# SysCV/LiDAR_snow_sim

Hardware: AMD Instinct MI355X
Metric: augmented points/s/GPU (64x2048 sweep, 2.5 mm/h); HBM roofline % -- value: rows resident in HBM when the clock starts (device-resident API: augment_batch on CUDA tensors); with H2D of the rows and D2H of the results inside the clock: value_pcie_inclusive (higher is better)
Workload: dtype f64

## Files before the change

lidar_snow_sim_amd/csrc/sg_common.h:

```cpp
#pragma once
#include <stddef.h>
#include <stdint.h>

#define SG_PI 3.141592653589793
#define SG_TWO_PI (2 * SG_PI)
#define SG_RBINS 1230
#define SG_NBINS 2048
#define SG_BIN_MARGIN 1e-6
#define SG_BEAM_MARGIN 1e-9
#define SG_TBL_STRIDE 16
#define SG_BLKREC 8
#define SG_HITS_UNDECIDED 0x40000000
#define SG_MAX_LASERS 256
#define SG_LCAP 63
#define SG_TILE 1024

struct SgEntry {
    double phi;
    double x, y, r;
    double t0, t1;
    double rho;
    uint32_t flags;
    uint32_t src;
};
// ... 51 lines not shown
    const void *srows;
    const int32_t *frame_unsorted;
    const SgTable *frame_tables;
    const SgLasers *las;
    const double *rgrid;
    double beam_div_deg;
    uint32_t *rec;
    uint32_t *rec_q;
    void *rng;
    int32_t *status;
    int32_t *tier_hint;
    unsigned long long *diff2;
    int32_t exact_math;
    int32_t n_cls;
    int32_t cls_cap[SG_MAX_CLASSES];
    const int32_t *seg_blk;
    const int64_t *seg_start;
    const int32_t *seg_cnt;
    const int32_t *seg_frame;
    const int32_t *seg_n;
    const int32_t *seg_of_blk;
    int64_t grid_blocks;
    int32_t q_chunk;
    int64_t blk_lo, blk_hi;
    const int32_t *chunk_blk;
    int32_t chunk;
    uint32_t *dq;
    int32_t *dq_g;
    uint16_t *dq_sc;
    unsigned long long *qn;
    int2_t *pw_items;
    int32_t *pw_count;
    int2_t *pw_items1;
    int32_t front_max;
    int64_t n_regions_ub;
    int32_t blk_rows;
    int32_t kp_lds_quarters;
    int64_t dq_n;
    int32_t *tier_list;
    int32_t *tier_info;
    int64_t tier_stride;
    int32_t *tier_sparse;
    int32_t *tn, *tbase;
    int32_t cls;
    int32_t work_lo, work_hi;
    int32_t work_hint;
    int32_t *redo_list;
    int32_t *redo_cnt;
    double *tq;
    uint16_t *tq_sc;
    int32_t tq_cap;
    double *ov;
    uint16_t *ov_sc;
    int32_t ov_cap;
    int32_t ov_list;
    double *h_lists;
    int32_t h_cap, h_lanes;
    int32_t *dbg_count;
    double *dbg_rj;
    double *dbg_ratio;
    int32_t dbg_cap;
};

struct SgFov {
    int32_t enabled;
    int32_t reserved_;
// ... 130 lines not shown
```

lidar_snow_sim_amd/csrc/sg_queue.h:

```cpp
#pragma once
#include "sg_beam.h"

#ifndef SG_DQ_ROW_HEADER
#define SG_DQ_ROW_HEADER 1
#endif
#if defined(__HIP_DEVICE_COMPILE__)
#define SG_DQ_RECORD(entries, w) (sg_gptr(entries) + ((w) & 0x3fffffffu))
#else
#define SG_DQ_RECORD(entries, w) ((entries) + ((w) & 0x3fffffffu))
#endif

__host__ __device__ __forceinline__ constexpr int sg_dq_hdr(int elem_size) { return SG_DQ_ROW_HEADER ? elem_size / 4 : 2; }
__host__ __device__ __forceinline__ constexpr int sg_dq_slot_words(int lmax, int hdr) { return 2 * hdr + lmax; }
__host__ __device__ __forceinline__ int64_t sg_dq_cell(int64_t slot, int plane, int lmax, int hdr)
{
    const int64_t group = (slot >> 6) * (int64_t)(64 * sg_dq_slot_words(lmax, hdr));
    const int c = (int)(slot & 63);
    return plane < 2 ? group + (int64_t)((plane * 64 + c) * hdr) : group + (int64_t)(128 * hdr + (plane - 2) * 64 + c);
}

template <typename T>
__host__ __device__ __forceinline__ void sg_dq_store_header(uint32_t *q, int64_t slot, int lmax, T d_t, T theta_t)
{
    constexpr int H = sg_dq_hdr((int)sizeof(T));
    using S = std::conditional_t<H == 2, double, float>;
    *reinterpret_cast<S *>(q + sg_dq_cell(slot, 0, lmax, H)) = (S)d_t;
    *reinterpret_cast<S *>(q + sg_dq_cell(slot, 1, lmax, H)) = (S)theta_t;
}
template <typename T>
__host__ __device__ __forceinline__ void sg_dq_store_word(uint32_t *q, int64_t slot, int lmax, int j, uint32_t w)
{
    q[sg_dq_cell(slot, 2 + j, lmax, sg_dq_hdr((int)sizeof(T)))] = w;
}

template <typename T>
__host__ __device__ __forceinline__ void sg_dq_load_header(const uint32_t *q, int64_t slot, int lmax, double &d, double &theta_c)
{
    constexpr int H = sg_dq_hdr((int)sizeof(T));
    using S = std::conditional_t<H == 2, double, float>;
    d = (double)*reinterpret_cast<const S *>(q + sg_dq_cell(slot, 0, lmax, H));
    theta_c = (double)*reinterpret_cast<const S *>(q + sg_dq_cell(slot, 1, lmax, H));
}
template <typename T>
__host__ __device__ __forceinline__ uint32_t sg_dq_load_word(const uint32_t *q, int64_t slot, int lmax, int j)
{
    return q[sg_dq_cell(slot, 2 + j, lmax, sg_dq_hdr((int)sizeof(T)))];
}

__host__ __device__ __forceinline__ void sg_dq_resolve(uint32_t w, const SgEntry *__restrict__ entries, double theta_r, double theta_l, double &a1, double &a2,
                                                       double &rho)
{
// ... 32 lines not shown
```

lidar_snow_sim_amd/csrc/snowgpu_batch.cpp:

```cpp
#include "sg_host.h"
#include "sg_launch.h"
#include "sg_queue.h"

static int sync_tables(snowgpu_ctx *ctx)
{
    if (!ctx->tables_dirty) return SNOWGPU_OK;
    const size_t n = std::max<size_t>(ctx->tables.size(), 1);
    if (n > ctx->d_tables_cap) {
        if (ctx->d_tables) { (void)hipStreamSynchronize(ctx->stream); (void)hipFree(ctx->d_tables); }
        HIPCHK(ctx, hipMalloc((void **)&ctx->d_tables, n * sizeof(SgTable)));
        ctx->d_tables_cap = n;
    }
    std::vector<SgTable> h(n);
    for (size_t i = 0; i < ctx->tables.size(); ++i) h[i] = ctx->tables[i].desc;
    HIPCHK(ctx, hipMemcpy(ctx->d_tables, h.data(), n * sizeof(SgTable), hipMemcpyHostToDevice));
    ctx->tables_dirty = false;
    return SNOWGPU_OK;
}

static void choose_tiers(const snowgpu_ctx *ctx, double beam_div_deg, int tiers[4], int *n_tiers)
{
    const double expect = (double)ctx->max_flakes * (beam_div_deg * (SG_PI / 180.0)) / SG_TWO_PI;
    int first = expect <= 24.0 ? 4 : (expect <= 48.0 ? 8 : (expect <= 96.0 ? 16 : SG_LCAP));
    if (ctx->first_tier_override == 4 || ctx->first_tier_override == 8 || ctx->first_tier_override == 16 ||
// ... 138 lines not shown
    const size_t regions = std::max<size_t>((size_t)b.n_frames * 256, n / q_chunk + 2);
    const size_t zero_words = 3 * regions + 2 * (size_t)b.n_frames + 8;
    ENSURE(ctx, ctx->qn, zero_words);
    ENSURE(ctx, ctx->tbase, SG_MAX_CLASSES * regions);
    bool seg_small = false;
    if (use_seg) {
        const int se = sg_launch_segments_small(b.frame_off, b.n_frames, ctx->tile_base.p, max_tiles, b.table_ids, R->h_las.n, (int)R->tables.size(), first_block,
                                                ctx->seg_blk.p, ctx->seg_start.p, ctx->seg_cnt.p, ctx->seg_frame.p, ctx->seg_n.p, ctx->seg_of_blk.p,
                                                ctx->chunk_blk.p, R->d_tables, ctx->frame_tables.p, ctx->qn.p, (int64_t)zero_words, st);
        if (se > 0) return fail(ctx, SNOWGPU_E_HIP, std::string("segment launch: ") + hipGetErrorString((hipError_t)se));
        seg_small = se == 0;
    }
    if (!seg_small) {
        HIPCHK(ctx, hipEventRecord(ctx->ev_fork, st));
        HIPCHK(ctx, hipStreamWaitEvent(s_aux, ctx->ev_fork, 0));
        int e = 0;
        if (!use_seg) e = sg_launch_resolve_tables(R->d_tables, (int)R->tables.size(), b.table_ids, n_ft, ctx->frame_tables.p, s_aux);
        if (e) return fail(ctx, SNOWGPU_E_HIP, std::string("table resolve launch: ") + hipGetErrorString((hipError_t)e));
        if (use_seg) {
            e = sg_launch_segments(b.frame_off, b.n_frames, ctx->tile_base.p, max_tiles, b.table_ids, R->h_las.n, (int)R->tables.size(), first_block,
                                   ctx->seg_tbl_cnt.p, ctx->seg_tbl_base.p, ctx->seg_blk.p, ctx->seg_start.p, ctx->seg_cnt.p, ctx->seg_frame.p,
                                   ctx->seg_n.p, ctx->seg_of_blk.p, ctx->chunk_blk.p, R->d_tables, ctx->frame_tables.p, s_aux);
            if (e) return fail(ctx, SNOWGPU_E_HIP, std::string("segment launch: ") + hipGetErrorString((hipError_t)e));
        }
        HIPCHK(ctx, hipEventRecord(ctx->ev_join, s_aux));
    }
    if (!b.perm) {
        int e = sg_launch_sort(b.rows, b.dtype, b.frame_off, b.n_frames, b.n_total, ctx->tile_hist.p, ctx->tile_base.p,
                               ctx->rank.p, ctx->keep.p, ctx->perm.p, b.status, max_tiles, nullptr, nullptr,
                               ctx->tile_unsorted.p, ctx->frame_unsorted.p, ctx->srows.p, b.want_perm ? 1 : 0, 2, st);
        if (e) return fail(ctx, SNOWGPU_E_HIP, std::string("sort launch: ") + hipGetErrorString((hipError_t)e));
    }
    ENSURE(ctx, ctx->rec, n);
    ENSURE(ctx, ctx->rec_q, n);
    ENSURE(ctx, ctx->rng, n * esz);
    ENSURE(ctx, ctx->keep, n);
    ENSURE(ctx, ctx->tier_list, n * (size_t)n_tiers);
    ENSURE(ctx, ctx->tier_sparse, n * (size_t)n_tiers);
    ENSURE(ctx, ctx->ctile_cnt, (size_t)b.n_frames * (size_t)max_tiles + 1);
    ENSURE(ctx, ctx->ctile_base, (size_t)b.n_frames * (size_t)max_tiles + 1);
    SgBeamArgs a{};
    a.rows = b.rows; a.frame_off = b.frame_off; a.n_frames = b.n_frames; a.n_total = b.n_total; a.perm = perm;
    a.srows = ctx->srows.p; a.frame_unsorted = ctx->frame_unsorted.p;
    a.uniform_rows = (b.uniform_rows > 0 && b.n_total < ((int64_t)1 << 31)) ? b.uniform_rows : 0;
    a.inv_uniform_rows = a.uniform_rows > 0 ? 1.0f / (float)a.uniform_rows : 0.0f;
    a.las = R->d_las; a.frame_tables = ctx->frame_tables.p;
    a.rgrid = R->d_rgrid; a.beam_div_deg = b.beam_div_deg; a.rec = ctx->rec.p; a.rec_q = ctx->rec_q.p;
    a.status = b.status;
    a.rng = ctx->rng.p;
    a.dbg_count = b.dbg_count; a.dbg_rj = b.dbg_rj; a.dbg_ratio = b.dbg_ratio; a.dbg_cap = b.dbg_cap;
    a.exact_math = R->exact_math;
    const int n_cls = n_tiers;
    const bool tier_rows = (R->tier_rows < 0 ? b.n_total <= ((int64_t)1 << 19) : R->tier_rows == 1) && R->tier_cap_override <= 0;
    const int h_lanes = 256;
    const int h_cap = (int)std::min<uint32_t>(std::max<uint32_t>(R->max_flakes, 64u), 8192u);
    a.n_cls = n_cls;
    for (int k = 0; k + 1 < n_cls; ++k) a.cls_cap[k] = tiers[k + 1];
    a.cls_cap[n_cls - 1] = h_cap;
    ENSURE(ctx, ctx->h_lists, (size_t)4 * (size_t)(h_cap + 1) * (size_t)h_lanes);
    a.h_lists = ctx->h_lists.p; a.h_cap = h_cap; a.h_lanes = h_lanes;
    a.tier_list = ctx->tier_list.p; a.tier_stride = b.n_total; a.tier_sparse = ctx->tier_sparse.p;
    if (tier_rows) {
        ENSURE(ctx, ctx->redo_list, n * (size_t)n_tiers);
        a.redo_list = ctx->redo_list.p;
    }
    const bool use_ov = tiers[0] < SG_OV_CAP && n_cls >= 2 && !tier_rows &&
                        R->tier_cap_override <= 0 && n * SG_OV_STRIDE * sizeof(double) <= ((size_t)40 << 30);
    int64_t tq_caps[SG_MAX_CLASSES] = {0, 0, 0, 0};
    for (int k = 0; k + 1 < n_cls && !tier_rows; ++k) {
        if (use_ov && tiers[k + 1] <= SG_OV_CAP) continue;
        tq_caps[k] = tier_queue_cap(R, tiers[k + 1], b.n_total);
        ENSURE(ctx, ctx->tq[k], ((size_t)tq_caps[k] + 64) * (3 * (size_t)tiers[k + 1] + 2));
        ENSURE(ctx, ctx->tq_sc[k], (size_t)tq_caps[k]);
    }
    a.q_chunk = (int32_t)q_chunk;
    {
        const size_t slot_words = (size_t)sg_dq_slot_words(tiers[0], sg_dq_hdr(b.dtype == 0 ? 4 : 8));
        if (n * slot_words * sizeof(uint32_t) > ((size_t)64 << 30))
            return fail(ctx, SNOWGPU_E_INVALID, "batch too large for the dict queue of this table density: split it");
        if (b.n_frames >= (1 << 22)) return fail(ctx, SNOWGPU_E_INVALID, "too many frames in one batch");
        ENSURE(ctx, ctx->dq, (n + 64) * slot_words);
        ENSURE(ctx, ctx->dq_g, n);
        ENSURE(ctx, ctx->dq_sc, n);
        if (!seg_small) HIPCHK(ctx, hipMemsetAsync(ctx->qn.p, 0, sizeof(unsigned long long) * zero_words, st));
        a.tn = (int32_t *)(ctx->qn.p + regions); a.tbase = ctx->tbase.p;
        a.diff2 = ctx->qn.p + 3 * regions;
        int32_t *small = (int32_t *)(ctx->qn.p + 3 * regions + (size_t)b.n_frames);
        a.tier_info = small; a.pw_count = small + 8; a.redo_cnt = small + 12;
        a.dq = ctx->dq.p; a.dq_g = ctx->dq_g.p; a.dq_sc = ctx->dq_sc.p; a.qn = ctx->qn.p; a.dq_n = b.n_total;
        const int lanes = first_block < 64 ? first_block : 64;
        a.n_regions_ub = use_seg ? (int64_t)b.n_frames * 256 : (b.n_total + a.q_chunk - 1) / a.q_chunk;
        a.blk_rows = first_block;
        a.kp_lds_quarters = 2;
        const size_t items_cap = n / (size_t)lanes + 2 * (size_t)a.n_regions_ub + 64;
        ENSURE(ctx, ctx->pw_items, 2 * items_cap);
        a.pw_items = ctx->pw_items.p;
        a.pw_items1 = (R->few > 0 && !b.dbg_count && lanes == 64) ? ctx->pw_items.p + items_cap : nullptr;
        a.front_max = a.pw_items1 ? std::min(R->few, std::min(3, tiers[0])) : 1;
    }
    if (use_ov) {
        ENSURE(ctx, ctx->ov, (n + 256) * SG_OV_STRIDE);
        ENSURE(ctx, ctx->ov_sc, n + 256);
        a.ov = ctx->ov.p; a.ov_sc = ctx->ov_sc.p; a.ov_cap = SG_OV_CAP;
    }
    if (use_seg) {
        a.seg_blk = ctx->seg_blk.p; a.seg_start = ctx->seg_start.p; a.seg_cnt = ctx->seg_cnt.p; a.seg_frame = ctx->seg_frame.p;
        a.seg_n = ctx->seg_n.p; a.seg_of_blk = ctx->seg_of_blk.p; a.chunk_blk = ctx->chunk_blk.p;
    }
    const bool few_first = a.pw_items1 && !serial && b.n_total > ((int64_t)1 << 19);
    bool heavy_tail = false;
    if (few_first && n_cls >= 3 && ctx->tier_hint_d) {
        const volatile int32_t *hint = ctx->tier_hint_h;
        long tail = 0;
        for (int k = 2; k < n_cls && k < SG_MAX_CLASSES; ++k) tail += hint[k];
        heavy_tail = R->heavy_tail < 0 ? (tail >= 4096 && tail * 22 > (long)hint[1]) : R->heavy_tail == 1;
        a.tier_hint = ctx->tier_hint_d;
    }
    if (!seg_small) HIPCHK(ctx, hipStreamWaitEvent(st, ctx->ev_join, 0));
    const bool timed = ctx->prof && ctx->ev_used < (int)ctx->ev_start.size();
    if (timed) { HIPCHK(ctx, hipEventRecord(ctx->ev_start[(size_t)ctx->ev_used], st)); ctx->prof_stream = st; }
    int e = 0;
    {
        const int64_t lin_blocks = (b.n_total + first_block - 1) / first_block;
        if (use_seg) {
            a.chunk = 0;
            a.grid_blocks = total_blocks_ub + b.max_frame / first_block + 2;
        } else {
            a.blk_lo = 0; a.blk_hi = lin_blocks;
            a.grid_blocks = lin_blocks;
        }
        e = sg_launch_beams(&a, b.dtype, tiers[0], 1, st);
// ... 144 lines not shown
```

lidar_snow_sim_amd/csrc/snowgpu_kernels.hip:

```cpp
#include <hip/hip_runtime.h>
#include <algorithm>
#include "sg_beam.h"
#include "sg_few.h"
#include "sg_queue.h"
#include "sg_kutil.h"
#include "sg_launch.h"

#ifndef SG_NB4
#define SG_NB4 4
#endif
#ifndef SG_KP_WIN
#define SG_KP_WIN 3
#endif
#ifndef SG_FP_WAVES
#define SG_FP_WAVES 6
#endif
#ifndef SG_FP_WAVES_SEG
#define SG_FP_WAVES_SEG 7
#endif
#ifndef SG_NB_TIERS
#define SG_NB_TIERS 4
#endif
#ifndef SG_KP_THREE_MAX
#define SG_KP_THREE_MAX 16
// ... 209 lines not shown
                tier_k = k;
                pending = true;
            }
        } else if (o.range_error) {
            atomicCAS(&a.status[0], 0, 4 );
            atomicCAS(&a.status[1], -1, (int32_t)g);
        }
    }
    if constexpr (!LIST) {
        if (__ballot(tier_k >= 0)) {
            for (int k = 0; k < a.n_cls; ++k) {
                const unsigned long long m = __ballot(tier_k == k);
                if (!m) continue;
                const int leader = __ffsll((long long)m) - 1;
                int base = 0;
                if ((tid & 63) == leader) base = atomicAdd(&a.tn[(int64_t)__builtin_amdgcn_readfirstlane(region) * SG_MAX_CLASSES + k], (int)__popcll(m));
                base = __shfl(base, leader);
                if (tier_k == k) a.tier_sparse[(int64_t)k * a.tier_stride + q_base + base + (int)__popcll(m & sg_lanemask_lt())] = (int32_t)g;
            }
        }
    }
    if constexpr (DICT) {
        auto hand_over = [&](uint32_t *q, int64_t slot) {
            sg_dq_store_header<T>(q, slot, LMAX, d_t, theta_t);
            const uint32_t *s_w = reinterpret_cast<const uint32_t *>(s_a1);
            if constexpr (LMAX <= 4) {
#pragma unroll
                for (int j = 0; j < LMAX; ++j)
                    if (j < L) sg_dq_store_word<T>(q, slot, LMAX, j, s_w[j * BLOCK + tid]);
            } else {
                for (int j = 0; j < L; ++j) sg_dq_store_word<T>(q, slot, LMAX, j, s_w[j * BLOCK + tid]);
            }
        };
        const bool front = o.has_power && L <= a.front_max, back = o.has_power && L > a.front_max;
        const unsigned long long mf = __ballot(front), mb = __ballot(back);
        if (mf | mb) {
            const int leader = __ffsll((long long)(mf | mb)) - 1;
            unsigned long long base = 0;
            if ((tid & 63) == leader)
                base = atomicAdd(&a.qn[__builtin_amdgcn_readfirstlane(region)], (unsigned long long)__popcll(mf) | ((unsigned long long)__popcll(mb) << 32));
            const unsigned blo = __shfl((unsigned)(base & 0xffffffffull), leader), bhi = __shfl((unsigned)(base >> 32), leader);
            if (o.has_power) {
                const int64_t slot = front ? q_base + (int)blo + (int)__popcll(mf & sg_lanemask_lt())
                                           : q_base + q_size - 1 - ((int)bhi + (int)__popcll(mb & sg_lanemask_lt()));
                hand_over(a.dq, slot);
                a.dq_g[slot] = (int32_t)g;
                a.dq_sc[slot] = (uint16_t)(L | (ch << 8));
                rec = SG_REC_SLOT | (uint32_t)slot;
            }
        }
    } else {
        constexpr int NB = LMAX <= 4 ? 4 : 8;
        if (o.has_power) {
            double best = 0.0;
            int k_best = 0;
            if (a.exact_math) sg_lane_power<BLOCK, true, NB, LMAX>(o.n_flakes, a.rgrid, s_a1, s_a2, s_rho, s_ratio, tid, best, k_best);
            else sg_lane_power<BLOCK, false, NB, LMAX>(o.n_flakes, a.rgrid, s_a1, s_a2, s_rho, s_ratio, tid, best, k_best);
            if constexpr (SgReal<T>::is_f32) d_t = sqrtf((px * px + py * py) + pz * pz);
            else d_t = sqrt((px * px + py * py) + pz * pz);
            sg_beam_decide((double)d_t, ch, a.las, best, k_best, o);
            rec = sg_pack_record(o);
        }
        sg_add_diff2(a.diff2, live, f, (long long)o.diff2);
    }
    if constexpr (DICT) {
        if (live && !pending && rec == 0u && act && a.rng) rec = rec_clear;
    }
    if (live && !pending) a.rec[g] = rec;
    } while (LIST && (chunk += stride) < work_n);
}

template <typename T, int LMAX>
__global__ __launch_bounds__(256, 4) void k_tier_scan_direct(SgBeamArgs a)
{
    constexpr int P = SG_QPLANES(LMAX);
    if constexpr (LMAX > 16) __builtin_amdgcn_s_setprio(3);
    const int n_las = a.las->n;
// ... 45 lines not shown
                a.dbg_rj[(int64_t)g * a.dbg_cap] = (double)d_t;
                a.dbg_ratio[(int64_t)g * a.dbg_cap] = sg_clear_beam_ratio(geo.theta_c, a.beam_div_deg);
            }
        } else {
            q[0] = (double)d_t; q[64] = geo.theta_c;
            a.tq_sc[slot] = (uint16_t)(hits | (ch << 8));
        }
    }
}

__device__ __forceinline__ bool sg_region(const SgBeamArgs &a, int r, int n_regions_ub, int64_t &q_base, int &q_size, int &f1)
{
    const int64_t lo = a.chunk_blk ? a.chunk_blk[a.chunk] : a.blk_lo, hi = a.chunk_blk ? a.chunk_blk[a.chunk + 1] : a.blk_hi;
    bool mine = false;
    q_base = 0; q_size = 0; f1 = 0;
    if (a.seg_blk) {
        if (r < a.seg_n[0]) {
            const int64_t b0 = a.seg_blk[r];
            mine = b0 >= lo && b0 < hi;
            if (mine) { q_base = a.seg_start[r]; q_size = a.seg_cnt[r]; f1 = (a.seg_frame[r] & 0x3fffff) + 1; }
        }
    } else if (r < n_regions_ub) {
        q_base = (int64_t)r * a.q_chunk;
        const int64_t b0 = q_base / a.blk_rows;
        mine = q_base < a.n_total && b0 >= lo && b0 < hi;
        if (mine) q_size = (int)(a.n_total - q_base < a.q_chunk ? a.n_total - q_base : a.q_chunk);
    }
    return mine;
}

__global__ __launch_bounds__(256) void k_power_plan(SgBeamArgs a, int lanes, int lanes_back, int n_regions_ub)
{
    const int r = blockIdx.x * 256 + threadIdx.x;
    int n_items = 0, nf = 0, nb = 0, q_size = 0, f1 = 0;
    int64_t q_base = 0;
    const bool mine = sg_region(a, r, n_regions_ub, q_base, q_size, f1);
    for (int k = 0; k < a.n_cls; ++k) {
        const int c = mine ? a.tn[(int64_t)r * SG_MAX_CLASSES + k] : 0;
        int inc = c;
        for (int o = 1; o < 64; o <<= 1) { const int v = __shfl_up(inc, o); if ((int)(threadIdx.x & 63) >= o) inc += v; }
        const int total = __shfl(inc, 63);
        int base = 0;
        if ((threadIdx.x & 63) == 63 && total > 0) base = atomicAdd(&a.tier_info[k], total);
        base = __shfl(base, 63) + inc - c;
        if (mine) a.tbase[(int64_t)r * SG_MAX_CLASSES + k] = base;
    }
    int n_one = 0;
    if (mine) {
        const unsigned long long c = a.qn[r];
        nf = (int)(c & 0xffffffffull); nb = (int)(c >> 32);
        n_one = (nf + lanes - 1) / lanes;
        n_items = (nb + lanes_back - 1) / lanes_back;
        if (!a.pw_items1) { n_items += n_one; n_one = 0; }
    }
    auto reserve = [&](int n, int32_t *counter) {
        int inc = n;
        for (int o = 1; o < 64; o <<= 1) { const int v = __shfl_up(inc, o); if ((int)(threadIdx.x & 63) >= o) inc += v; }
        const int total = __shfl(inc, 63);
        int b = 0;
        if ((threadIdx.x & 63) == 63 && total > 0) b = atomicAdd(counter, total);
        return __shfl(b, 63) + inc - n;
    };
    int base = reserve(n_items, a.pw_count);
    if (a.pw_items1) {
        int base1 = reserve(n_one, a.pw_count + 1);
        for (int k = 0; k < nf; k += lanes)
            a.pw_items1[base1++] = make_int2((int)(q_base + k), (nf - k < lanes ? nf - k : lanes) | (f1 << 10));
    } else {
        for (int k = 0; k < nf; k += lanes)
            a.pw_items[base++] = make_int2((int)(q_base + k), (nf - k < lanes ? nf - k : lanes) | (f1 << 10));
    }
    for (int k = 0; k < nb; k += lanes_back)
        a.pw_items[base++] = make_int2((int)(q_base + q_size - nb + k), (nb - k < lanes_back ? nb - k : lanes_back) | (f1 << 10));
}

__global__ __launch_bounds__(256) void k_tier_gather(SgBeamArgs a, int n_regions_ub)
{
    const int r = blockIdx.x * 4 + (int)(threadIdx.x >> 6), lane = (int)(threadIdx.x & 63);
    if (blockIdx.x == 0 && threadIdx.x < SG_MAX_CLASSES) a.status[2 + threadIdx.x] = a.tier_info[threadIdx.x];
    if (blockIdx.x == 0 && threadIdx.x < SG_MAX_CLASSES && a.tier_hint) a.tier_hint[threadIdx.x] = a.tier_info[threadIdx.x];
    if (blockIdx.x == 0 && threadIdx.x == 0 && a.tier_hint) a.tier_hint[SG_MAX_CLASSES] = (int32_t)((a.n_total >> 10) + 1);
    int q_size = 0, f1 = 0;
    int64_t q_base = 0;
    if (!sg_region(a, r, n_regions_ub, q_base, q_size, f1)) return;
    for (int k = 0; k < a.n_cls; ++k) {
        const int c = a.tn[(int64_t)r * SG_MAX_CLASSES + k];
        if (c == 0) continue;
        const int32_t *src = a.tier_sparse + (int64_t)k * a.tier_stride + q_base;
        int32_t *dst = a.tier_list + (int64_t)k * a.tier_stride + a.tbase[(int64_t)r * SG_MAX_CLASSES + k];
        for (int i = lane; i < c; i += 64) dst[i] = src[i];
    }
}

__device__ __forceinline__ const SgEntry *sg_dq_entries(const SgBeamArgs &a, int f, int ch)
{
    return a.frame_tables[(int64_t)f * a.las->n + ch].entries;
}

template <typename T, int LMAX, int BLOCK, bool LISTQ>
__device__ __forceinline__ void sg_kp_item(const SgBeamArgs &a, char *smem, const int ov_list, const int64_t work_off,
                                           const int start, const int cnt, const int item_f)
{
    constexpr int LANES = BLOCK < 64 ? BLOCK : 64;
    constexpr int WIN = BLOCK < 64 ? 1 : SG_KP_WIN;
    constexpr int P = SG_QPLANES(LMAX);
    double *s_a1 = (double *)smem;
// ... 223 lines not shown
    constexpr int THREADS = BLOCK < 64 ? 64 : BLOCK, WAVES = THREADS / 64, LANES = BLOCK < 64 ? BLOCK : 64;
    constexpr int WIN = BLOCK < 64 ? 1 : SG_KP_WIN;
    extern __shared__ __attribute__((aligned(16))) char smem[];
    if constexpr (LMAX > 16) __builtin_amdgcn_s_setprio(3);
    const int tid = threadIdx.x;
    int64_t work_n = 0, work_off = 0;
    int n_items;
    const int step = (int)gridDim.x * WAVES;
    int item_slots = LANES * WIN;
    if (LISTQ) {
        work_n = a.tier_info[a.cls];
        if (work_n > a.work_hi) work_n = a.work_hi;
        work_off = (int64_t)a.cls * a.tier_stride;
        if (WIN > 1 && work_n <= (int64_t)step * LANES) item_slots = LANES;
        n_items = (int)((work_n + item_slots - 1) / item_slots);
    } else {
        n_items = *a.pw_count;
    }
    for (int i = (int)blockIdx.x * WAVES + __builtin_amdgcn_readfirstlane(tid >> 6); i < n_items; i += step) {
        int start, cnt, item_f = -1;
        if (LISTQ) {
            start = i * item_slots;
            cnt = (int)(work_n - start < item_slots ? work_n - start : item_slots);
        } else {
            const int2 d = a.pw_items[i];
            start = __builtin_amdgcn_readfirstlane(d.x);
            const int dy = __builtin_amdgcn_readfirstlane(d.y);
            cnt = dy & 1023; item_f = (dy >> 10) - 1;
        }
        sg_kp_item<T, LMAX, BLOCK, LISTQ>(a, smem, a.ov_list, work_off, start, cnt, item_f);
    }
}

template <typename T, int N>
__global__ __launch_bounds__(256, 4) void k_power_few(SgBeamArgs a, int lmax)
{
    __shared__ double s_amp[N + 1][256], s_rho[N + 1][256], s_best[256];
    __shared__ int s_win[N + 1][256], s_zone[N + 1][256], s_k[256];
    __shared__ int s_mark[256];
    const int tid = (int)threadIdx.x, lane = tid & 63, wbase = tid & ~63;
    const int n_items = a.pw_count[1];
    const int step = (int)gridDim.x * 4;
    for (int i = (int)blockIdx.x * 4 + __builtin_amdgcn_readfirstlane(tid >> 6); i < n_items; i += step) {
        const int2 it = a.pw_items1[i];
        const int start = __builtin_amdgcn_readfirstlane(it.x), dy = __builtin_amdgcn_readfirstlane(it.y);
        const int cnt = dy & 1023, item_f = (dy >> 10) - 1;
        const bool live = lane < cnt;
        const int64_t slot = (int64_t)start + lane;
        SgBeamOut o;
        o.overflow = 0; o.range_error = 0; o.diff2 = 0.0; o.has_power = 0; o.n_flakes = 0; o.n_hits = 0; o.label = 0; o.new_i = 0; o.k_best = 0;
        int f = 0, ch = 0, S = 0, g = 0;
        SgFew<N> P{};
        int zone[N + 1], n = 0;
#pragma unroll
        for (int z = 0; z <= N; ++z) zone[z] = 0;
        if (live) {
            const unsigned sc = a.dq_sc[slot];
            double d, tc;
            sg_dq_load_header<T>(a.dq, slot, lmax, d, tc);
            uint32_t w[N];
#pragma unroll
            for (int j = 0; j < N; ++j) w[j] = sg_dq_load_word<T>(a.dq, slot, lmax, j);
            ch = (int)(sc >> 8);
            g = a.dq_g[slot];
            f = item_f >= 0 ? item_f : sg_frame_of(a, g);
            const SgEntry *ent = sg_dq_entries(a, f, ch);
            double th_r, th_l, a1[N], a2[N], rho[N];
            sg_beam_limits(tc, a.beam_div_deg, th_r, th_l);
            sg_dq_resolve_all<N>(w, (int)(sc & 255u), ent, th_r, th_l, a1, a2, rho);
            S = sg_few_prep<T, N>(d, tc, (int)(sc & 255u), a1, a2, rho, ch, a.las, a.beam_div_deg, P, o);
            if (S) {
                int ka, kb;
                sg_few_zone<N, 0>(P, 0.0, ka, kb);
                if (kb >= ka) { zone[0] = ka | ((kb - ka + 1) << 16); n += kb - ka + 1; }
                if constexpr (N >= 2) { sg_few_zone<N, 1>(P, 0.0, ka, kb); if (kb >= ka) { zone[1] = ka | ((kb - ka + 1) << 16); n += kb - ka + 1; } }
                if constexpr (N >= 3) { sg_few_zone<N, 2>(P, 0.0, ka, kb); if (kb >= ka) { zone[2] = ka | ((kb - ka + 1) << 16); n += kb - ka + 1; } }
                sg_few_zone<N, N>(P, 0.0, ka, kb);
// ... 48 lines not shown
                sm = a.exact_math ? sg_few_bin<true, N>(amp, rho, k0, k1, s_amp[N][col], s_rho[N][col], tw & 0xffff, (int)((unsigned)tw >> 16), k, a.rgrid)
                                  : sg_few_bin<false, N>(amp, rho, k0, k1, s_amp[N][col], s_rho[N][col], tw & 0xffff, (int)((unsigned)tw >> 16), k, a.rgrid);
                kk = k; oo = ow;
            }
            sg_fold_runs(sm, kk, oo);
            const int on = sg_dpp<0x130, 0xf>(oo, oo);
            if (valid && (lane == 63 || on != oo)) {
                volatile double *vb = s_best;
                volatile int *vk = s_k;
                const int col = wbase + oo;
                const double b0 = vb[col];
                const int kc = vk[col];
                if (sm > b0 || (sm == b0 && kk < kc)) { vb[col] = sm; vk[col] = kk; }
            }
        }
        asm volatile("s_waitcnt lgkmcnt(0)" ::: "memory");
        if (live) {
            uint32_t rec = 0;
            if (S) {
                const double best = ((volatile double *)s_best)[tid];
                const int k_best = ((volatile int *)s_k)[tid];
                if (o.range_error) {
                    atomicCAS(&a.status[0], 0, 4 );
                    atomicCAS(&a.status[1], -1, g);
                }
                sg_beam_decide(P.d, ch, a.las, best, k_best, o);
                rec = sg_pack_record(o);
            }
            a.rec_q[slot] = rec;
        }
        sg_add_diff2(a.diff2, live, f, live ? (long long)o.diff2 : 0);
        asm volatile("s_waitcnt lgkmcnt(0)" ::: "memory");
    }
}

template <typename T>
__global__ __launch_bounds__(64) void k_beams_huge(SgBeamArgs a)
{
    const int tid = (int)(blockIdx.x * 64 + threadIdx.x);
    const int rstride = a.h_lanes;
    const size_t col = (size_t)(a.h_cap + 1) * (size_t)a.h_lanes;
    double *s_a1 = a.h_lists, *s_a2 = s_a1 + col, *s_rho = s_a2 + col, *s_ratio = s_rho + col;
    const int n_las = a.las->n;
    int64_t work_n = a.tier_info[a.cls];
    const int64_t work_off = (int64_t)a.cls * a.tier_stride;
    int64_t chunk = (int64_t)blockIdx.x * 64;
    if (chunk >= work_n) return;
    do {
    const bool live = chunk + threadIdx.x < work_n;
    int64_t g = 0;
    int f = 0;
    SgBeamOut o;
    o.overflow = 0; o.range_error = 0; o.diff2 = 0.0; o.has_power = 0; o.n_flakes = 0; o.n_hits = 0; o.label = 0; o.new_i = 0; o.k_best = 0;
    if (live) {
        g = a.tier_list[work_off + chunk + threadIdx.x];
        f = sg_frame_of(a, g);
        const T *row = sg_row<T>(a, f, g);
        const T px = row[0], py = row[1], pz = row[2];
        const int ch = (int)row[4];
        const SgTable tab = a.frame_tables[(int64_t)f * n_las + ch];
        int32_t *dc = a.dbg_count ? a.dbg_count + g : nullptr;
        double *drj = a.dbg_count ? a.dbg_rj + g * a.dbg_cap : nullptr;
        double *dra = a.dbg_count ? a.dbg_ratio + g * a.dbg_cap : nullptr;
        sg_beam<T, 0, 0>(px, py, pz, ch, tab, a.las, a.beam_div_deg, s_a1, s_a2, s_rho, s_ratio, tid, o, a.dbg_cap, dc, drj,
                                dra, a.exact_math != 0, rstride, a.h_cap);
        uint32_t rec = 0;
// ... 44 lines not shown
    if (blocks == 0) return 0;
    hipLaunchKernelGGL((k_beams<T, LMAX, BLOCK, LIST, DICT, SEG>), dim3(blocks), dim3(THREADS), lds, st, *a);
    SG_CHECK_LAUNCH();
    return 0;
}

template <typename T, int LMAX, int BLOCK, bool LISTQ>
static int launch_power_t(const SgBeamArgs *a, hipStream_t st, bool plan_only = false, hipEvent_t ev_few = nullptr, int which = 3)
{
    const size_t lds = sizeof(double) * ((size_t)BLOCK * ((SG_KP_THREE_MAX > 0 && LMAX <= SG_KP_THREE_MAX && LMAX >= SG_KP_THREE_MIN) ? 3 : 4) * (LMAX + 1));
    static bool attr_set[64] = {};
    if (int e = sg_set_lds(k_power<T, LMAX, BLOCK, LISTQ>, lds, attr_set)) return e;
    constexpr int THREADS = BLOCK < 64 ? 64 : BLOCK, LANES = BLOCK < 64 ? BLOCK : 64;
    const int cus = sg_cu_count();
    unsigned per_cu = (unsigned)std::min<size_t>(32 * 64 / THREADS, std::max<size_t>(1, (size_t)(160 * 1024) / lds));
    if (!LISTQ && a->kp_lds_quarters > 0 && a->kp_lds_quarters < 4) per_cu = std::max(1u, per_cu * (unsigned)a->kp_lds_quarters / 4u);
    int64_t blocks = (int64_t)cus * per_cu;
    int64_t items_ub = LISTQ ? ((int64_t)a->work_hi + LANES - 1) / LANES : (a->n_total + LANES - 1) / LANES + 2 * a->n_regions_ub;
    if (LISTQ && a->work_hint > 0) items_ub = std::min<int64_t>(items_ub, (4 * (int64_t)a->work_hint + LANES - 1) / LANES + 8);
    blocks = std::min<int64_t>(blocks, (items_ub + THREADS / 64 - 1) / (THREADS / 64));
    if (blocks <= 0) return 0;
    if (!LISTQ) {
        const unsigned pg = (unsigned)((a->n_regions_ub + 255) / 256);
        if (pg == 0) return 0;
        const int64_t back_est = a->n_total / 10;
        const int lanes_back = (BLOCK < 64 || back_est <= (int64_t)blocks * (THREADS / 64) * LANES * 5 / 2) ? LANES : LANES * SG_KP_WIN;
        if (plan_only) {
            hipLaunchKernelGGL(k_power_plan, dim3(pg), dim3(256), 0, st, *a, LANES, lanes_back, (int)a->n_regions_ub);
            SG_CHECK_LAUNCH();
            return 0;
        }
        if (a->pw_items1 && (which & 1)) {
            hipStream_t s1 = st;
            const unsigned g1 = (unsigned)std::min<int64_t>((int64_t)cus * 4, (a->n_total / LANES + a->n_regions_ub + 3) / 4);
            if (g1 > 0) {
                if (a->front_max == 1) hipLaunchKernelGGL((k_power_few<T, 1>), dim3(g1), dim3(256), 0, s1, *a, LMAX);
                else if (a->front_max == 2) hipLaunchKernelGGL((k_power_few<T, 2>), dim3(g1), dim3(256), 0, s1, *a, LMAX);
                else hipLaunchKernelGGL((k_power_few<T, 3>), dim3(g1), dim3(256), 0, s1, *a, LMAX);
            }
            SG_CHECK_LAUNCH();
            if (ev_few && hipEventRecord(ev_few, st) != hipSuccess) return (int)hipGetLastError();
        }
    }
    if (!(which & 2)) return 0;
    hipLaunchKernelGGL((k_power<T, LMAX, BLOCK, LISTQ>), dim3((unsigned)blocks), dim3(THREADS), lds, st, *a);
    SG_CHECK_LAUNCH();
    return 0;
}

extern "C" int sg_launch_tier_scan(const SgBeamArgs *a, int dtype, int lmax, void *stream)
{
    const int64_t n = (int64_t)a->work_hi - a->work_lo;
    if (n <= 0) return 0;
    int64_t want = (n + 255) / 256;
    if (a->work_hint > 0) want = std::min<int64_t>(want, (4 * (int64_t)a->work_hint + 255) / 256 + 8);
    const unsigned blocks = (unsigned)std::min<int64_t>(want, (int64_t)sg_cu_count() * 8);
    return sg_by_dtype_tier<false>(dtype, lmax, [&](auto t, auto tier) {
        hipLaunchKernelGGL((k_tier_scan_direct<decltype(t), decltype(tier)::LMAX>), dim3(blocks), dim3(256), 0, (hipStream_t)stream, *a);
        SG_CHECK_LAUNCH();
        return 0;
    });
}

extern "C" int sg_beams_block(int lmax)
{
    return sg_by_tier<true>(lmax, [](auto tier) { return decltype(tier)::BLOCK; });
}

extern "C" int sg_launch_beams(const SgBeamArgs *a, int dtype, int lmax, int direct, void *stream)
{
    hipStream_t st = (hipStream_t)stream;
// ... 44 lines not shown
```

Baseline: 10.39 billion.

## Split dict queue into one-flake and few-flake lists for specialized power kernels

Beams whose front list holds one scatterer are now queued separately from those with two or three, using a second queue region (dq_n2 offset) and a three-way packed counter. The plan kernel emits separate work-item lists, and k_power_few processes single-flake items with the N=1 code path instead of the wider N=2/3 path. This avoids spending wider per-beam work and LDS on beams that need only one scatterer. The cost is roughly double the queue and rec_q allocations, extra packing logic, and either an extra launch or a combined kernel.

Result: no change. 10.45 billion (median of 6 runs) (+0.6%).

```diff
diff --git a/lidar_snow_sim_amd/csrc/sg_common.h b/lidar_snow_sim_amd/csrc/sg_common.h
--- a/lidar_snow_sim_amd/csrc/sg_common.h
+++ b/lidar_snow_sim_amd/csrc/sg_common.h
@@ -107,6 +107,8 @@
     int2_t *pw_items;
     int32_t *pw_count;
     int2_t *pw_items1;
+    int2_t *pw_items_one;
+    int64_t dq_n2;
     int32_t front_max;
     int64_t n_regions_ub;
     int32_t blk_rows;
diff --git a/lidar_snow_sim_amd/csrc/sg_queue.h b/lidar_snow_sim_amd/csrc/sg_queue.h
--- a/lidar_snow_sim_amd/csrc/sg_queue.h
+++ b/lidar_snow_sim_amd/csrc/sg_queue.h
@@ -17,6 +17,55 @@
     const int64_t group = (slot >> 6) * (int64_t)(64 * sg_dq_slot_words(lmax, hdr));
     const int c = (int)(slot & 63);
     return plane < 2 ? group + (int64_t)((plane * 64 + c) * hdr) : group + (int64_t)(128 * hdr + (plane - 2) * 64 + c);
+}
+
+#ifndef SG_FEW_SPLIT
+#define SG_FEW_SPLIT 1
+#endif
+enum { SG_DQ_ONE = 0, SG_DQ_FEW = 1, SG_DQ_BACK = 2 };
+#define SG_DQ_SPLIT_BITS 21
+struct SgDqCounts { int one, few, back; };
+
+__host__ __device__ __forceinline__ constexpr int64_t sg_dq_n2(int64_t n_total) { return (n_total + 63) & ~(int64_t)63; }
+__host__ __device__ __forceinline__ constexpr int64_t sg_dq_split_base(bool items1, int front_max, int64_t n_total)
+{
+    return (SG_FEW_SPLIT && items1 && front_max >= 2 && sg_dq_n2(n_total) + n_total + 64 < ((int64_t)1 << 31)) ? sg_dq_n2(n_total) : 0;
+}
+__host__ __device__ __forceinline__ constexpr int64_t sg_dq_slots(int64_t dq_n2, int64_t n_total) { return dq_n2 > 0 ? dq_n2 + n_total : n_total; }
+__host__ __device__ __forceinline__ constexpr bool sg_dq_split(int64_t dq_n2, int q_size) { return dq_n2 > 0 && q_size < (1 << SG_DQ_SPLIT_BITS); }
+__host__ __device__ __forceinline__ constexpr int sg_dq_kind(bool split, int L, int front_max)
+{
+    return L > front_max ? SG_DQ_BACK : (split && L >= 2 ? SG_DQ_FEW : SG_DQ_ONE);
+}
+__host__ __device__ __forceinline__ constexpr unsigned long long sg_dq_pack(bool split, int n_one, int n_few, int n_back)
+{
+    return split ? (unsigned long long)n_one | ((unsigned long long)n_few << SG_DQ_SPLIT_BITS) | ((unsigned long long)n_back << (2 * SG_DQ_SPLIT_BITS))
+                 : (unsigned long long)(n_one + n_few) | ((unsigned long long)n_back << 32);
+}
+__host__ __device__ __forceinline__ SgDqCounts sg_dq_unpack(bool split, unsigned long long w)
+{
+    constexpr unsigned long long M = (1ull << SG_DQ_SPLIT_BITS) - 1ull;
+    SgDqCounts c;
+    if (split) { c.one = (int)(w & M); c.few = (int)((w >> SG_DQ_SPLIT_BITS) & M); c.back = (int)((w >> (2 * SG_DQ_SPLIT_BITS)) & M); }
+    else { c.one = (int)(w & 0xffffffffull); c.few = 0; c.back = (int)(w >> 32); }
+    return c;
+}
+__host__ __device__ __forceinline__ int64_t sg_dq_place(int kind, int64_t q_base, int q_size, int64_t dq_n2, int index)
+{
+    return kind == SG_DQ_BACK ? q_base + q_size - 1 - index : (kind == SG_DQ_FEW ? dq_n2 + q_base + index : q_base + index);
+}
+struct SgDqItem { int64_t start; int count; };
+__host__ __device__ __forceinline__ int sg_dq_items(int kind, const SgDqCounts &c, int lanes, int lanes_back)
+{
+    return kind == SG_DQ_BACK ? (c.back + lanes_back - 1) / lanes_back : ((kind == SG_DQ_FEW ? c.few : c.one) + lanes - 1) / lanes;
+}
+__host__ __device__ __forceinline__ SgDqItem sg_dq_item(int kind, const SgDqCounts &c, int64_t q_base, int q_size, int64_t dq_n2, int lanes, int lanes_back, int i)
+{
+    const int per = kind == SG_DQ_BACK ? lanes_back : lanes, n = kind == SG_DQ_BACK ? c.back : (kind == SG_DQ_FEW ? c.few : c.one), k = i * per;
+    SgDqItem it;
+    it.start = kind == SG_DQ_BACK ? q_base + q_size - n + k : (kind == SG_DQ_FEW ? dq_n2 + q_base + k : q_base + k);
+    it.count = n - k < per ? n - k : per;
+    return it;
 }
 
 template <typename T>
diff --git a/lidar_snow_sim_amd/csrc/snowgpu_batch.cpp b/lidar_snow_sim_amd/csrc/snowgpu_batch.cpp
--- a/lidar_snow_sim_amd/csrc/snowgpu_batch.cpp
+++ b/lidar_snow_sim_amd/csrc/snowgpu_batch.cpp
@@ -194,7 +194,6 @@
         if (e) return fail(ctx, SNOWGPU_E_HIP, std::string("sort launch: ") + hipGetErrorString((hipError_t)e));
     }
     ENSURE(ctx, ctx->rec, n);
-    ENSURE(ctx, ctx->rec_q, n);
     ENSURE(ctx, ctx->rng, n * esz);
     ENSURE(ctx, ctx->keep, n);
     ENSURE(ctx, ctx->tier_list, n * (size_t)n_tiers);
@@ -207,7 +206,7 @@
     a.uniform_rows = (b.uniform_rows > 0 && b.n_total < ((int64_t)1 << 31)) ? b.uniform_rows : 0;
     a.inv_uniform_rows = a.uniform_rows > 0 ? 1.0f / (float)a.uniform_rows : 0.0f;
     a.las = R->d_las; a.frame_tables = ctx->frame_tables.p;
-    a.rgrid = R->d_rgrid; a.beam_div_deg = b.beam_div_deg; a.rec = ctx->rec.p; a.rec_q = ctx->rec_q.p;
+    a.rgrid = R->d_rgrid; a.beam_div_deg = b.beam_div_deg; a.rec = ctx->rec.p;
     a.status = b.status;
     a.rng = ctx->rng.p;
     a.dbg_count = b.dbg_count; a.dbg_rj = b.dbg_rj; a.dbg_ratio = b.dbg_ratio; a.dbg_cap = b.dbg_cap;
@@ -238,27 +237,33 @@
     a.q_chunk = (int32_t)q_chunk;
     {
         const size_t slot_words = (size_t)sg_dq_slot_words(tiers[0], sg_dq_hdr(b.dtype == 0 ? 4 : 8));
-        if (n * slot_words * sizeof(uint32_t) > ((size_t)64 << 30))
+        const int lanes = first_block < 64 ? first_block : 64;
+        const bool few_kernel = R->few > 0 && !b.dbg_count && lanes == 64;
+        a.front_max = few_kernel ? std::min(R->few, std::min(3, tiers[0])) : 1;
+        a.dq_n2 = sg_dq_split_base(few_kernel, a.front_max, b.n_total);
+        const size_t q_slots = (size_t)sg_dq_slots(a.dq_n2, b.n_total);
+        if (q_slots * slot_words * sizeof(uint32_t) > ((size_t)64 << 30))
             return fail(ctx, SNOWGPU_E_INVALID, "batch too large for the dict queue of this table density: split it");
         if (b.n_frames >= (1 << 22)) return fail(ctx, SNOWGPU_E_INVALID, "too many frames in one batch");
-        ENSURE(ctx, ctx->dq, (n + 64) * slot_words);
-        ENSURE(ctx, ctx->dq_g, n);
-        ENSURE(ctx, ctx->dq_sc, n);
+        ENSURE(ctx, ctx->dq, (q_slots + 64) * slot_words);
+        ENSURE(ctx, ctx->dq_g, q_slots);
+        ENSURE(ctx, ctx->dq_sc, q_slots);
+        ENSURE(ctx, ctx->rec_q, q_slots);
+        a.rec_q = ctx->rec_q.p;
         if (!seg_small) HIPCHK(ctx, hipMemsetAsync(ctx->qn.p, 0, sizeof(unsigned long long) * zero_words, st));
         a.tn = (int32_t *)(ctx->qn.p + regions); a.tbase = ctx->tbase.p;
         a.diff2 = ctx->qn.p + 3 * regions;
         int32_t *small = (int32_t *)(ctx->qn.p + 3 * regions + (size_t)b.n_frames);
         a.tier_info = small; a.pw_count = small + 8; a.redo_cnt = small + 12;
         a.dq = ctx->dq.p; a.dq_g = ctx->dq_g.p; a.dq_sc = ctx->dq_sc.p; a.qn = ctx->qn.p; a.dq_n = b.n_total;
-        const int lanes = first_block < 64 ? first_block : 64;
-        a.n_regions_ub = use_seg ? (int64_t)b.n_frames * 256 : (b.n_total + a.q_chunk - 1) / a.q_chunk;
+        a.n_regions_ub =use_seg ? (int64_t)b.n_frames * 256 : (b.n_total + a.q_chunk - 1) / a.q_chunk;
         a.blk_rows = first_block;
         a.kp_lds_quarters = 2;
         const size_t items_cap = n / (size_t)lanes + 2 * (size_t)a.n_regions_ub + 64;
-        ENSURE(ctx, ctx->pw_items, 2 * items_cap);
+        ENSURE(ctx, ctx->pw_items, (a.dq_n2 > 0 ? 3 : 2) * items_cap);
         a.pw_items = ctx->pw_items.p;
-        a.pw_items1 = (R->few > 0 && !b.dbg_count && lanes == 64) ? ctx->pw_items.p + items_cap : nullptr;
-        a.front_max = a.pw_items1 ? std::min(R->few, std::min(3, tiers[0])) : 1;
+        a.pw_items1 = few_kernel ? ctx->pw_items.p + items_cap : nullptr;
+        a.pw_items_one = a.dq_n2 > 0 ? ctx->pw_items.p + 2 * items_cap : nullptr;
     }
     if (use_ov) {
         ENSURE(ctx, ctx->ov, (n + 256) * SG_OV_STRIDE);
diff --git a/lidar_snow_sim_amd/csrc/snowgpu_kernels.hip b/lidar_snow_sim_amd/csrc/snowgpu_kernels.hip
--- a/lidar_snow_sim_amd/csrc/snowgpu_kernels.hip
+++ b/lidar_snow_sim_amd/csrc/snowgpu_kernels.hip
@@ -265,17 +265,21 @@
                 for (int j = 0; j < L; ++j) sg_dq_store_word<T>(q, slot, LMAX, j, s_w[j * BLOCK + tid]);
             }
         };
-        const bool front = o.has_power && L <= a.front_max, back = o.has_power && L > a.front_max;
-        const unsigned long long mf = __ballot(front), mb = __ballot(back);
-        if (mf | mb) {
-            const int leader = __ffsll((long long)(mf | mb)) - 1;
+        const bool split = sg_dq_split(a.dq_n2, q_size);
+        const int kind = o.has_power ? sg_dq_kind(split, L, a.front_max) : -1;
+        const unsigned long long mk = __ballot(kind >= 0);
+        if (mk) {
+            const unsigned long long mf = __ballot(kind == SG_DQ_FEW), mb = __ballot(kind == SG_DQ_BACK), mo = mk & ~(mf | mb);
+            const int leader = __builtin_amdgcn_readfirstlane(__ffsll((long long)mk) - 1);
             unsigned long long base = 0;
             if ((tid & 63) == leader)
-                base = atomicAdd(&a.qn[__builtin_amdgcn_readfirstlane(region)], (unsigned long long)__popcll(mf) | ((unsigned long long)__popcll(mb) << 32));
-            const unsigned blo = __shfl((unsigned)(base & 0xffffffffull), leader), bhi = __shfl((unsigned)(base >> 32), leader);
+                base = atomicAdd(&a.qn[__builtin_amdgcn_readfirstlane(region)], sg_dq_pack(split, (int)__popcll(mo), (int)__popcll(mf), (int)__popcll(mb)));
+            const SgDqCounts before = sg_dq_unpack(split, ((unsigned long long)(unsigned)__builtin_amdgcn_readlane((int)(base >> 32), leader) << 32)
+                                                              | (unsigned)__builtin_amdgcn_readlane((int)(base & 0xffffffffull), leader));
             if (o.has_power) {
-                const int64_t slot = front ? q_base + (int)blo + (int)__popcll(mf & sg_lanemask_lt())
-                                           : q_base + q_size - 1 - ((int)bhi + (int)__popcll(mb & sg_lanemask_lt()));
+                const unsigned long long mine = kind == SG_DQ_BACK ? mb : (kind == SG_DQ_FEW ? mf : mo);
+                const int index = (kind == SG_DQ_BACK ? before.back : (kind == SG_DQ_FEW ? before.few : before.one)) + (int)__popcll(mine & sg_lanemask_lt());
+                const int64_t slot = sg_dq_place(kind, q_base, q_size, a.dq_n2, index);
                 hand_over(a.dq, slot);
                 a.dq_g[slot] = (int32_t)g;
                 a.dq_sc[slot] = (uint16_t)(L | (ch << 8));
@@ -387,7 +391,7 @@
 __global__ __launch_bounds__(256) void k_power_plan(SgBeamArgs a, int lanes, int lanes_back, int n_regions_ub)
 {
     const int r = blockIdx.x * 256 + threadIdx.x;
-    int n_items = 0, nf = 0, nb = 0, q_size = 0, f1 = 0;
+    int n_items = 0, q_size = 0, f1 = 0;
     int64_t q_base = 0;
     const bool mine = sg_region(a, r, n_regions_ub, q_base, q_size, f1);
     for (int k = 0; k < a.n_cls; ++k) {
@@ -400,13 +404,16 @@
         base = __shfl(base, 63) + inc - c;
         if (mine) a.tbase[(int64_t)r * SG_MAX_CLASSES + k] = base;
     }
-    int n_one = 0;
+    int n_one = 0, n_few = 0, n_back = 0;
+    SgDqCounts c{0, 0, 0};
+    bool split = false;
     if (mine) {
-        const unsigned long long c = a.qn[r];
-        nf = (int)(c & 0xffffffffull); nb = (int)(c >> 32);
-        n_one = (nf + lanes - 1) / lanes;
-        n_items = (nb + lanes_back - 1) / lanes_back;
-        if (!a.pw_items1) { n_items += n_one; n_one = 0; }
+        split = sg_dq_split(a.dq_n2, q_size);
+        c = sg_dq_unpack(split, a.qn[r]);
+        n_one = sg_dq_items(SG_DQ_ONE, c, lanes, lanes_back);
+        n_few = sg_dq_items(SG_DQ_FEW, c, lanes, lanes_back);
+        n_back = sg_dq_items(SG_DQ_BACK, c, lanes, lanes_back);
+        n_items = a.pw_items1 ? n_back : n_back + n_one;
     }
     auto reserve = [&](int n, int32_t *counter) {
         int inc = n;
@@ -416,17 +423,25 @@
         if ((threadIdx.x & 63) == 63 && total > 0) b = atomicAdd(counter, total);
         return __shfl(b, 63) + inc - n;
     };
+    auto emit = [&](int2 *dst, int at, int kind, int n) {
+        for (int i = 0; i < n; ++i) {
+            const SgDqItem it = sg_dq_item(kind, c, q_base, q_size, a.dq_n2, lanes, lanes_back, i);
+            dst[at + i] = make_int2((int)it.start, it.count | (f1 << 10));
+        }
+        return at + n;
+    };
     int base = reserve(n_items, a.pw_count);
     if (a.pw_items1) {
-        int base1 = reserve(n_one, a.pw_count + 1);
-        for (int k = 0; k < nf; k += lanes)
-            a.pw_items1[base1++] = make_int2((int)(q_base + k), (nf - k < lanes ? nf - k : lanes) | (f1 << 10));
+        const int base1 = reserve(split ? n_few : n_one, a.pw_count + 1);
+        emit(a.pw_items1, base1, split ? SG_DQ_FEW : SG_DQ_ONE, split ? n_few : n_one);
+        if (a.dq_n2 > 0) {
+            const int base2 = reserve(split ? n_one : 0, a.pw_count + 2);
+            if (split) emit(a.pw_items_one, base2, SG_DQ_ONE, n_one);
+        }
     } else {
-        for (int k = 0; k < nf; k += lanes)
-            a.pw_items[base++] = make_int2((int)(q_base + k), (nf - k < lanes ? nf - k : lanes) | (f1 << 10));
-    }
-    for (int k = 0; k < nb; k += lanes_back)
-        a.pw_items[base++] = make_int2((int)(q_base + q_size - nb + k), (nb - k < lanes_back ? nb - k : lanes_back) | (f1 << 10));
+        base = emit(a.pw_items, base, SG_DQ_ONE, n_one);
+    }
+    emit(a.pw_items, base, SG_DQ_BACK, n_back);
 }
 
 __global__ __launch_bounds__(256) void k_tier_gather(SgBeamArgs a, int n_regions_ub)
@@ -716,17 +731,22 @@
     }
 }
 
-template <typename T, int N>
-__global__ __launch_bounds__(256, 4) void k_power_few(SgBeamArgs a, int lmax)
-{
-    __shared__ double s_amp[N + 1][256], s_rho[N + 1][256], s_best[256];
-    __shared__ int s_win[N + 1][256], s_zone[N + 1][256], s_k[256];
-    __shared__ int s_mark[256];
+template <int N>
+struct SgFewLds {
+    double amp[N + 1][256], rho[N + 1][256], best[256];
+    int win[N + 1][256], zone[N + 1][256], k[256];
+    int mark[256];
+};
+
+template <typename T, int N, int NL>
+__device__ __forceinline__ void sg_few_item(const SgBeamArgs &a, const int lmax, SgFewLds<NL> &lds, const int2 it)
+{
+    static_assert(N <= NL, "the block's cells hold NL + 1 scatterers per beam");
+    auto &s_amp = lds.amp; auto &s_rho = lds.rho; auto &s_best = lds.best;
+    auto &s_win = lds.win; auto &s_zone = lds.zone; auto &s_k = lds.k;
+    int *s_mark = lds.mark;
     const int tid = (int)threadIdx.x, lane = tid & 63, wbase = tid & ~63;
-    const int n_items = a.pw_count[1];
-    const int step = (int)gridDim.x * 4;
-    for (int i = (int)blockIdx.x * 4 + __builtin_amdgcn_readfirstlane(tid >> 6); i < n_items; i += step) {
-        const int2 it = a.pw_items1[i];
+    {
         const int start = __builtin_amdgcn_readfirstlane(it.x), dy = __builtin_amdgcn_readfirstlane(it.y);
         const int cnt = dy & 1023, item_f = (dy >> 10) - 1;
         const bool live = lane < cnt;
@@ -841,6 +861,20 @@
         sg_add_diff2(a.diff2, live, f, live ? (long long)o.diff2 : 0);
         asm volatile("s_waitcnt lgkmcnt(0)" ::: "memory");
     }
+}
+
+template <typename T, int N, int LISTS>
+__global__ __launch_bounds__(256, 4) void k_power_few(SgBeamArgs a, int lmax)
+{
+    static_assert(LISTS == 1 || LISTS == 3 || (LISTS == 2 && N == 1), "the one-flake items take the N = 1 code");
+    __shared__ SgFewLds<N> lds;
+    const int n_front = (LISTS & 1) ? a.pw_count[1] : 0, n_items = n_front + ((LISTS & 2) ? a.pw_count[2] : 0);
+    const int step = (int)gridDim.x * 4;
+    int i = (int)blockIdx.x * 4 + __builtin_amdgcn_readfirstlane((int)threadIdx.x >> 6);
+    if constexpr ((LISTS & 1) != 0)
+        for (; i < n_front; i += step) sg_few_item<T, N, N>(a, lmax, lds, a.pw_items1[i]);
+    if constexpr ((LISTS & 2) != 0)
+        for (; i < n_items; i += step) sg_few_item<T, 1, N>(a, lmax, lds, a.pw_items_one[i - n_front]);
 }
 
 template <typename T>
@@ -951,11 +985,24 @@
         }
         if (a->pw_items1 && (which & 1)) {
             hipStream_t s1 = st;
-            const unsigned g1 = (unsigned)std::min<int64_t>((int64_t)cus * 4, (a->n_total / LANES + a->n_regions_ub + 3) / 4);
+            const unsigned g1 = (unsigned)std::min<int64_t>((int64_t)cus * 4, (a->n_total / LANES + (a->dq_n2 > 0 ? 2 : 1) * a->n_regions_ub + 3) / 4);
             if (g1 > 0) {
-                if (a->front_max == 1) hipLaunchKernelGGL((k_power_few<T, 1>), dim3(g1), dim3(256), 0, s1, *a, LMAX);
-                else if (a->front_max == 2) hipLaunchKernelGGL((k_power_few<T, 2>), dim3(g1), dim3(256), 0, s1, *a, LMAX);
-                else hipLaunchKernelGGL((k_power_few<T, 3>), dim3(g1), dim3(256), 0, s1, *a, LMAX);
+                if (a->dq_n2 > 0) {
+#if defined(SG_FEW_TWO_LAUNCHES)
+                    hipLaunchKernelGGL((k_power_few<T, 1, 2>), dim3(g1), dim3(256), 0, s1, *a, LMAX);
+                    if (a->front_max == 2) hipLaunchKernelGGL((k_power_few<T, 2, 1>), dim3(g1), dim3(256), 0, s1, *a, LMAX);
+                    else hipLaunchKernelGGL((k_power_few<T, 3, 1>), dim3(g1), dim3(256), 0, s1, *a, LMAX);
+#else
+                    if (a->front_max == 2) hipLaunchKernelGGL((k_power_few<T, 2, 3>), dim3(g1), dim3(256), 0, s1, *a, LMAX);
+                    else {
+                        hipLaunchKernelGGL((k_power_few<T, 3, 1>), dim3(g1), dim3(256), 0, s1, *a, LMAX);
+                        hipLaunchKernelGGL((k_power_few<T, 1, 2>), dim3(g1), dim3(256), 0, s1, *a, LMAX);
+                    }
+#endif
+                }
+                else if (a->front_max == 1) hipLaunchKernelGGL((k_power_few<T, 1, 1>), dim3(g1), dim3(256), 0, s1, *a, LMAX);
+                else if (a->front_max == 2) hipLaunchKernelGGL((k_power_few<T, 2, 1>), dim3(g1), dim3(256), 0, s1, *a, LMAX);
+                else hipLaunchKernelGGL((k_power_few<T, 3, 1>), dim3(g1), dim3(256), 0, s1, *a, LMAX);
             }
             SG_CHECK_LAUNCH();
             if (ev_few && hipEventRecord(ev_few, st) != hipSuccess) return (int)hipGetLastError();
```
